# Nablax/Path-Tracer-CUDA-OpenGL

Measured on AMD Instinct MI355X. Metric: Mray/s + ms/frame, bunny-in-Cornell 1920×1080 @1024spp, 1/2/4/8 MI355X, higher is better.
Workload: dtype f32

## Files before the change

### path-tracer-cuda-opengl_amd/csrc/pt_device.hip

```cpp
#include <hip/hip_runtime.h>

#include <algorithm>
#include <array>
#include <atomic>
#include <chrono>
#include <cfloat>
#include <cmath>
#include <cstdio>
#include <cstdlib>
#include <cstring>
#include <limits>
#include <type_traits>
#include <memory>
#include <string>
#include <vector>

#include "../host/pt_denoise_dev.hpp"
#include "../host/pt_error.hpp"
#include "../host/pt_host.hpp"
#include "../host/pt_inst_dev.hpp"
#include "../host/pt_instancing.hpp"
#include "../host/pt_wide8.hpp"
#include "../host/pt_wide_dev.hpp"
#include "pt.h"
// ... 74 lines not shown
    if (l == 0.0f) return f3(0.0f, 0.0f, 0.0f);
    return divs(v, l);
}
__device__ __forceinline__ float3 xyz(float4 v) { return f3(v.x, v.y, v.z); }

struct Xorwow {
    uint32_t d, v0, v1, v2, v3, v4;
    __device__ __forceinline__ uint32_t next() {
        uint32_t t = v0 ^ (v0 >> 2);
        v0 = v1; v1 = v2; v2 = v3; v3 = v4;
        v4 = __builtin_amdgcn_bitop3_b32(v4, v4 << 4, t ^ (t << 1), 0x96);
        d += 362437u;
        return v4 + d;
    }
    __device__ __forceinline__ float uniform() { return uniformOf(next()); }
    __device__ __forceinline__ float centered2() { return centered2Of(uniform()); }
    __device__ __forceinline__ float3 centered2x3() {
        uint32_t t0 = v0 ^ (v0 >> 2), t1 = v1 ^ (v1 >> 2), t2 = v2 ^ (v2 >> 2);
        asm volatile("" : "+v"(t0), "+v"(t1), "+v"(t2));
        uint32_t r0, r1;
        asm volatile("v_mov_b32 %0, %1" : "=v"(r0) : "v"(v3));
        asm volatile("v_mov_b32 %0, %1" : "=v"(r1) : "v"(v4));
        const uint32_t n0 = __builtin_amdgcn_bitop3_b32(v4, v4 << 4, t0 ^ (t0 << 1), 0x96);
        const uint32_t n1 = __builtin_amdgcn_bitop3_b32(n0, n0 << 4, t1 ^ (t1 << 1), 0x96);
        const uint32_t n2 = __builtin_amdgcn_bitop3_b32(n1, n1 << 4, t2 ^ (t2 << 1), 0x96);
        uint32_t x0 = n0 + (d + 362437u), x1 = n1 + (d + 2u * 362437u);
        asm volatile("" : "+v"(x0), "+v"(x1));
        d += 3u * 362437u;
        v0 = r0; v1 = r1; v2 = n0; v3 = n1; v4 = n2;
        return f3(centered2Of(uniformOf(x0)), centered2Of(uniformOf(x1)), centered2Of(uniformOf(n2 + d)));
    }
};

__device__ __forceinline__ Xorwow sampleStream(uint32_t k0, uint32_t k1, uint32_t sample, uint32_t pixel) {
    uint32_t c0 = sample, c1 = pixel, c2 = 0u, c3 = 0x53414D50u;
#pragma unroll 2
    for (int r = 0; r < 10; r++) {
        const uint64_t p0 = (uint64_t)0xD2511F53u * c0, p1 = (uint64_t)0xCD9E8D57u * c2;
        const uint32_t hi0 = (uint32_t)(p0 >> 32), lo0 = (uint32_t)p0;
        const uint32_t hi1 = (uint32_t)(p1 >> 32), lo1 = (uint32_t)p1;
        const uint32_t n0 = __builtin_amdgcn_bitop3_b32(hi1, c1, k0, 0x96), n2 = __builtin_amdgcn_bitop3_b32(hi0, c3, k1, 0x96);
        c0 = n0; c1 = lo1; c2 = n2; c3 = lo0;
        k0 += 0x9E3779B9u;
        k1 += 0xBB67AE85u;
    }
    return Xorwow{c3, c0, c1, c2, c3 ^ 0x6C078965u, c0 ^ c1 ^ 0x2545F491u};
}

struct SlabHit { bool hit; float lo; };

__host__ __device__ constexpr int nodeBoxIdx(int child, int axis, int isMax) { return 6 * child + 2 * axis + isMax; }

typedef float v2f __attribute__((ext_vector_type(2)));

__device__ __forceinline__ SlabHit slabPair(v2f X, v2f Y, v2f Z, float3 o, float3 inv, float tmin, float tmax) {
    const v2f tx = (X - o.x) * inv.x, ty = (Y - o.y) * inv.y, tz = (Z - o.z) * inv.z;
    float nx = inv.x < 0.0f ? tx.y : tx.x, fx = inv.x < 0.0f ? tx.x : tx.y;
    float ny = inv.y < 0.0f ? ty.y : ty.x, fy = inv.y < 0.0f ? ty.x : ty.y;
    float nz = inv.z < 0.0f ? tz.y : tz.x, fz = inv.z < 0.0f ? tz.x : tz.y;
    float lo = fmaxf(fmaxf(fmaxf(tmin, nx), ny), nz);
    float hi = fminf(fminf(fminf(tmax, fx), fy), fz);
    return SlabHit{!(hi < lo), lo};
}
struct SlabHit2 { SlabHit l, r; };
__device__ __forceinline__ SlabHit2 slabBoth(float4 a, float4 b, float4 q, float3 o, float3 inv, float tmin,
                                             float tmax) {
    const v2f lx = (v2f{a.x, a.y} - o.x) * inv.x, ly = (v2f{a.z, a.w} - o.y) * inv.y,
              lz = (v2f{b.x, b.y} - o.z) * inv.z;
    const v2f rx = (v2f{b.z, b.w} - o.x) * inv.x, ry = (v2f{q.x, q.y} - o.y) * inv.y,
              rz = (v2f{q.z, q.w} - o.z) * inv.z;
// ... 3 lines not shown
        const float lo = fmaxf(fmaxf(fmaxf(tmin, sx ? lx.y : lx.x), sy ? ly.y : ly.x), sz ? lz.y : lz.x);
        const float hi = fminf(fminf(fminf(tmax, sx ? lx.x : lx.y), sy ? ly.x : ly.y), sz ? lz.x : lz.y);
        h.l = SlabHit{!(hi < lo), lo};
    }
    {
        const float lo = fmaxf(fmaxf(fmaxf(tmin, sx ? rx.y : rx.x), sy ? ry.y : ry.x), sz ? rz.y : rz.x);
        const float hi = fminf(fminf(fminf(tmax, sx ? rx.x : rx.y), sy ? ry.x : ry.y), sz ? rz.x : rz.y);
        h.r = SlabHit{!(hi < lo), lo};
    }
    return h;
}
__device__ __forceinline__ SlabHit slabLeft(float4 a, float4 b, float3 o, float3 inv, float tmin, float tmax) {
    return slabPair(v2f{a.x, a.y}, v2f{a.z, a.w}, v2f{b.x, b.y}, o, inv, tmin, tmax);
}
__device__ __forceinline__ SlabHit slabRight(float4 b, float4 q, float3 o, float3 inv, float tmin, float tmax) {
    return slabPair(v2f{b.z, b.w}, v2f{q.x, q.y}, v2f{q.z, q.w}, o, inv, tmin, tmax);
}

struct Prim { float4 p0, p1, p2; };
__device__ __forceinline__ __amdgpu_buffer_rsrc_t rawRsrc(const void* base) {
    return __builtin_amdgcn_make_buffer_rsrc(const_cast<void*>(base), 0, -1 , 0x00020000);
}
template <int S>
__device__ __forceinline__ uint32_t shlOpaque(uint32_t x) {
    uint32_t t;
    asm("v_lshlrev_b32 %0, %1, %2" : "=v"(t) : "i"(S), "v"(x));
    return t;
}
__device__ __forceinline__ uint32_t mul80(uint32_t x) {
    if constexpr (pt::kW8NodeDwords == 32) return x << 7;
    return shlOpaque<6>(x) + (x << 4);
}
__device__ __forceinline__ uint32_t mul48(uint32_t x) { return shlOpaque<5>(x) + (x << 4); }
__device__ __forceinline__ float4 bload4(__amdgpu_buffer_rsrc_t r, uint32_t off) {
    return __builtin_bit_cast(float4, __builtin_amdgcn_raw_buffer_load_b128(r, off, 0, 0));
}

__device__ __forceinline__ Prim loadPrim(const DevScene& S, uint32_t k) {
    const float4* p = S.prims + 3 * (size_t)k;
    return Prim{p[0], p[1], p[2]};
}

__device__ __forceinline__ float primHitT(const Prim& q, bool sphere, float3 o, float3 d, float tmin, float closest) {
    if (sphere) {
        float3 oc = sub(o, xyz(q.p0));
        float r = q.p1.x;
        float a = len2(d);
        float half_b = dot3(oc, d);
        float cc = len2(oc) - r * r;
        float disc = half_b * half_b - a * cc;
        if (disc < 0.0f) return -1.0f;
        float sq = sqrtf(disc);
        float root = (-half_b - sq) / a;
        if (root < tmin || closest < root) {
            root = (-half_b + sq) / a;
            if (root < tmin || closest < root) return -1.0f;
        }
        return root;
    }
    const float3 v0 = xyz(q.p0);
    float3 e1 = sub(xyz(q.p1), v0), e2 = sub(xyz(q.p2), v0);
    float3 s1 = cross3(d, e2);
    float det = dot3(s1, e1);
    if (det == 0.0f) return -1.0f;
    float3 s = sub(o, v0);
    float3 s2 = cross3(s, e1);
// ... 74 lines not shown
                                         int& best, float& bestLo, bool leafBoxes, bool& redo, uint32_t keyHi = 0u) {
    const bool sph = SPH && __float_as_uint(q.p2.w) != 0u;
    const float t = primHitAny(q, sph, o, d, tmin);
    if (t >= 0.0f) {
        const int k = (int)(keyHi | __float_as_uint(q.p0.w));
        const bool none = best < 0, bSph = SPH && (best & (int)kSphereBit) != 0;
        const int bk = SPH ? best & (int)kPrimMask : best;
        const bool tie = sph ? (none || !bSph || k > bk) : (!none && !bSph && k < bk);
        redo = redo || (t >= closest && t < bestLo);
        if (t < closest || (t == closest && tie)) {
            bool take = true;
            float lo = -__builtin_inff();
            if (leafBoxes) {
                const SlabHit b = refLeafBox(q, sph, o, inv, tmin, __builtin_inff());
                take = b.hit && !(closest < b.lo);
                redo = redo || (b.hit && closest < b.lo);
                lo = t < b.lo ? b.lo : lo;
            }
            if (take) {
                closest = t;
                best = k | (sph ? (int)kSphereBit : 0);
                bestLo = lo;
            }
        }
    }
}

__device__ __forceinline__ float rcpRNWave(float x, uint64_t hasM) {
    if constexpr (!PT_FAST_RCP) return 1.0f / x;
    const uint32_t ex = (__float_as_uint(x) >> 23) & 0xffu;
    const uint64_t slowM = hasM & __ballot(ex - kRcpExpLo > kRcpExpHi - kRcpExpLo);
    float y = rcpNewton(x);
    if (__builtin_expect(slowM != 0, 0)) y = __builtin_amdgcn_inverse_ballot_w64(slowM) ? 1.0f / x : y;
    return y;
}
__device__ __forceinline__ void wideTestTri(const Prim& q, uint64_t hasM, float3 o, float3 d, float tmin, float& closest,
                                            int& best, float& t2) {
    const float3 v0 = xyz(q.p0), e1 = xyz(q.p1), e2 = xyz(q.p2);
    const float3 s1 = cross3(d, e2);
    const float det = dot3(s1, e1);
    const float3 s = sub(o, v0);
    const float3 s2 = cross3(s, e1);
    const float inv = rcpRNWave(det, hasM);
    const float t = dot3(s2, e2) * inv;
    const float b1 = dot3(s1, s) * inv;
    const float b2 = dot3(s2, d) * inv;
    const int k = (int)__float_as_uint(q.p0.w);
    const uint64_t rejM = __ballot(b1 >= 1.0f) | __ballot(b1 <= 0.0f) | __ballot(b2 >= 1.0f) | __ballot(b2 <= 0.0f) |
                          __ballot(b1 + b2 >= 1.0f);
    const uint64_t hitM = hasM & __ballot(det != 0.0f) & __ballot(t > tmin) & ~rejM;
    const uint64_t takeM = hitM & (__ballot(t < closest) | (__ballot(t == closest) & __ballot(k < best)));
    const float mid = __builtin_amdgcn_fmed3f(t, closest, t2);
    t2 = __builtin_amdgcn_inverse_ballot_w64(hitM) ? mid : t2;
    closest = __builtin_amdgcn_inverse_ballot_w64(takeM) ? t : closest;
    best = __builtin_amdgcn_inverse_ballot_w64(takeM) ? k : best;
}
__device__ __forceinline__ bool deferredRedo(float4 xy, float2 z, float3 o, float3 inv, float closest, float t2) {
    const SlabHit b = slabPair(v2f{xy.x, xy.y}, v2f{xy.z, xy.w}, v2f{z.x, z.y}, o, inv, 0.001f, __builtin_inff());
    return !b.hit || (closest < b.lo && t2 < b.lo);
}

template <bool MIX = false, bool DEC3 = false>
__device__ __forceinline__ uint32_t wideHits(uint4 n0, uint4 n1, uint4 n2, uint4 n3, uint4 n4, float3 o, float3 inv,
                                             uint32_t oct, float tmin, float tmax) {
    constexpr uint32_t kMixExp = MIX ? 24u : 0u;
    float ax, ay, az;
// ... 179 lines not shown
        const uint32_t lref = __float_as_uint(r.x), rref = __float_as_uint(r.y);
        int next = -1;
        if (from < 0) {
            const SlabHit hl = slabLeft(a, b, o, inv, tmin, closest);
            if (hl.hit && (lref & kLeafBit)) {
                const float t = primHitT(loadPrim(S, lref & kPrimMask), (lref & kSphereBit) != 0, o, d, tmin, closest);
                if (t >= 0.0f) { closest = t; best = (int)(lref & kPrimMask); }
            }
            const SlabHit hr = slabRight(b, q, o, inv, tmin, closest);
            if (hr.hit && (rref & kLeafBit)) {
                const float t = primHitT(loadPrim(S, rref & kPrimMask), (rref & kSphereBit) != 0, o, d, tmin, closest);
                if (t >= 0.0f) { closest = t; best = (int)(rref & kPrimMask); }
            }
            if (hr.hit && !(rref & kLeafBit)) next = (int)rref;
            else if (!(lref & kLeafBit) && slabLeft(a, b, o, inv, tmin, closest).hit) next = (int)lref;
        } else if ((uint32_t)from == rref && !(lref & kLeafBit) && slabLeft(a, b, o, inv, tmin, closest).hit) {
            next = (int)lref;
        }
        if (next >= 0) {
            node = next;
            from = -1;
        } else {
            if (node == 0) { finished = true; break; }
            from = node;
            node = S.iparent[node];
        }
    }
    if (!finished) atomicOr(S.err, 4u);
    return best;
}

struct HitRec { float3 p, n; int mat, obj; bool front; float4 m0; float ir; int type; };

__device__ __forceinline__ HitRec makeHitFrom(const float4* shade, int k, float t, float3 o, float3 d) {
    HitRec h;
    const float4* r = shade + 3 * (size_t)k;
    const float4 s0 = r[0], s1 = r[1], s2 = r[2];
    const uint32_t tf = __float_as_uint(s2.y);
    h.p = add(o, scale(t, d));
    float3 outward;
    if (tf >> 16) {
        outward = divs(sub(h.p, xyz(s0)), s0.w);
    } else {
        outward = xyz(s0);
    }
    h.front = dot3(d, outward) < 0.0f;
    h.n = h.front ? outward : neg(outward);
    h.mat = (int)__float_as_uint(s2.z);
    h.obj = (int)__float_as_uint(s2.w);
    h.m0 = s1;
    h.ir = s2.x;
    h.type = (int)(tf & 0xffffu);
    return h;
}
__device__ __forceinline__ HitRec makeHit(const DevScene& S, int k, float t, float3 o, float3 d) {
    return makeHitFrom(S.shade, k, t, o, d);
}

__device__ __forceinline__ float3 xformPoint(float4 r0, float4 r1, float4 r2, float3 p) {
    return f3(((r0.x * p.x + r0.y * p.y) + r0.z * p.z) + r0.w, ((r1.x * p.x + r1.y * p.y) + r1.z * p.z) + r1.w,
              ((r2.x * p.x + r2.y * p.y) + r2.z * p.z) + r2.w);
}
__device__ __forceinline__ float3 xformDir(float4 r0, float4 r1, float4 r2, float3 v) {
    return f3((r0.x * v.x + r0.y * v.y) + r0.z * v.z, (r1.x * v.x + r1.y * v.y) + r1.z * v.z,
              (r2.x * v.x + r2.y * v.y) + r2.z * v.z);
}
__device__ __forceinline__ HitRec makeHitInst(const DevScene& S, uint32_t key, float t, float3 o, float3 d, int& obj) {
    const uint32_t inst = key >> S.gBits, g = key & ((1u << S.gBits) - 1u);
    const float4* ir = S.winst + 4 * (size_t)inst;
    const float4 r0 = ir[0], r1 = ir[1], r2 = ir[2], ex = ir[3];
    const float4* r = S.wshade + 3 * (size_t)g;
    const float4 s0 = r[0], s1 = r[1], s2 = r[2];
    const uint32_t tf = __float_as_uint(s2.y);
    const bool ident = __float_as_uint(ex.y) == 1u, linIdent = __float_as_uint(ex.y) != 0u;
    HitRec h;
    h.p = add(o, scale(t, d));
    float3 outward;
// ... 569 lines not shown
        } else if (bidT < ks) { slice = bidT % P.splitWays; bidT /= P.splitWays; }
        else bidT -= ks - P.splitTiles;
    }
    int tile = (SAMPLE || crit) ? -1 : tileOf(P, bidT), nSamples = SAMPLE ? 0 : P.spp;
    int col = 0, lrow = 0;
    bool valid = false;
    uint32_t idx = 0u;
    if constexpr (!SAMPLE) {
        if (crit) {
            const int k = bidT * P.critLanes + lane;
            valid = lane < P.critLanes && k < P.nCrit;
            idx = valid ? P.critList[k] : 0u;
            col = (int)(idx % (uint32_t)P.width);
            lrow = (int)(idx / (uint32_t)P.width);
        } else {
            col = (tile % P.tiles_x) * 8 + (lane & 7);
            lrow = (tile / P.tiles_x) * 8 + (lane >> 3);
            valid = col < P.width && lrow < P.nrows && (slice < 0 || (lane * P.splitWays) / kWave == slice);
            idx = valid ? (uint32_t)lrow * (uint32_t)P.width + (uint32_t)col : 0u;
            if (CRITK && valid && P.critFlag && P.critFlag[idx]) valid = false;
        }
    }
    const unsigned long long tStart = __builtin_amdgcn_s_memrealtime();
    if (!SAMPLE && !crit && bidT < P.prioTiles) {
        if (P.prioLevel >= 3) __builtin_amdgcn_s_setprio(3);
        else if (P.prioLevel == 2) __builtin_amdgcn_s_setprio(2);
        else __builtin_amdgcn_s_setprio(1);
    }
    float fcol = (float)col;
    float frow = valid ? (float)globalRow(lrow, P.stripe_h, P.nparts, P.part) : 0.0f;
    const DevScene& S = P.S;
    const __amdgpu_buffer_rsrc_t nodeRsrc = rawRsrc(WIDE ? (const void*)S.wnodes : (const void*)S.nodes);
    uint32_t* my = stk + lane;
    uint32_t sRays = 0, sVisits = 0, sTris = 0, sSph = 0, sPaths = 0;
#ifdef PT_DIAG
    uint32_t itN = 0, itL = 0, itS = 0, sPops = 0, sRedo = 0;
    uint32_t sRedoMiss = 0;
    unsigned long long sSpecN = 0, sIdleN = 0;
    unsigned long long sHalf = 0, sParkT = 0;
    unsigned long long cycN = 0, cycL = 0, cycS = 0, cycH = 0;
    unsigned long long cycSh = 0, cycTk = 0, cycNp = 0, cycBr = 0;
#define PT_DIAG_ADD(v, x) (v) += (x)
#else
#define PT_DIAG_ADD(v, x) ((void)0)
#endif

    Xorwow g{};
    if constexpr (!SAMPLE) {
        if (valid) g = Xorwow{P.sd[idx], P.s0[idx], P.s1[idx], P.s2[idx], P.s3[idx], P.s4[idx]};
    }
    float3 sum = f3(0.0f, 0.0f, 0.0f), o = f3(0.0f, 0.0f, 0.0f), d = f3(0.0f, 0.0f, 1.0f);
    float3 inv = d, att = f3(1.0f, 1.0f, 1.0f);
    float closest = 0.0f;
    int best = -1, depthLeft = 0, sample = 0, node = -1, sp = 0, qn = 0;
    constexpr int LQ = (SAMPLE && !WIDE && STACK <= 32) ? PT_LEAF_QUEUE_SAMPLE : kLeafQ;
    uint32_t qref[LQ];
    float lq[LQ];
#pragma unroll
    for (int i = 0; i < LQ; i++) { qref[i] = 0u; lq[i] = 0.0f; }
    uint32_t ng = 0u, tgBase = 0u, tg = 0u, oct = 0u;
    float bestLo = 0.0f;
    const uint64_t allM = __ballot(true);
    uint64_t activeM = 0;
    uint32_t depthPaths = 0;
    uint32_t pxRays = 0;
    uint64_t needTaskM = SAMPLE ? allM : 0;
    uint32_t poolBase = 0u, poolLeft = 0u;


#define PT_BEGIN_RAY(SH)                                                                            \
    do {                                                                                          \
        const bool sh_ = NEE && (SH);                                                             \
        if constexpr (NEE) depthLeft -= sh_ ? 0 : 1;                                              \
        else depthLeft--;                                                                         \
        if constexpr (SAMPLE) {    \
            if (kargs()->measureCost)                                                             \
                __hip_atomic_fetch_add(&taskState[lane].w, 1u, __ATOMIC_RELAXED, __HIP_MEMORY_SCOPE_WORKGROUP); \
        }                                                                                         \
        closest = sh_ ? kShadowTmax : __builtin_inff();                                           \
        best = -1;                                                                                \
        sp = 0;                                                                                   \
        qn = 0;                                                                                   \
        if constexpr (CRITK) pxRays++;                                                            \
        if constexpr (WIDE) {                 \
            inv = f3(rcpRN(d.x), rcpRN(d.y), rcpRN(d.z));                                         \
            const uint32_t oc_ = (inv.x < 0.0f ? 1u : 0u) | (inv.y < 0.0f ? 2u : 0u) | (inv.z < 0.0f ? 4u : 0u); \
            oct = oc_;                                                                            \
            tg = 0u;                                                                              \
                    \
                   \
            if constexpr (TRI) bestLo = closest;                                                  \
            else bestLo = INST || kargs()->S.hasSpheres ? -__builtin_inff() : closest;            \
            ng = S.nprims > 0 ? (1u << oc_) : 0u;                                                 \
                 \
            if (!INST && ((kargs()->camFar && !sh_ && depthLeft + 1 == kargs()->max_depth) ||      \
                          (PT_WIDE_MIX && mixUnsafe(inv, kargs()->S.mixLim)))) {                   \
                ng = 0u;             \
                oct |= 8u;      \
            }                                                                                     \
            if (INST && kargs()->camFar && !sh_ && depthLeft + 1 == kargs()->max_depth) {          \
                     \
                const auto& K_ = *kargs();                                                        \
                (void)instEntry(K_.S.cx, K_.S.cy, K_.S.cz, K_.S.ext, o, d, inv);                   \
            }                                                                                     \
            if (CRITK && crit) PT_CRIT_TRACE();                                                    \
        } else if (S.nprims <= 1) {                                                               \
            node = -1;                                                                            \
            if (S.nprims == 1) {        \
                const float t1 = primHitT(loadPrim(S, 0), __float_as_uint(S.prims[2].w) != 0, o, d, \
                                          0.001f, closest);                                       \
                if (t1 >= 0.0f) { closest = t1; best = 0; }                                       \
            }                                                                                     \
        } else {                                                                                  \
            inv = f3(rcpRN(d.x), rcpRN(d.y), rcpRN(d.z));                                         \
            node = 0;                                                                             \
        }                                                                                         \
    } while (0)
#define PT_CRIT_TRACE()                                                                             \
    do {                                                                                          \
        const bool lb_ = S.nprims > 1;                                                            \
        bool sph_ = false;                                                                        \
        if constexpr (!TRI) sph_ = kargs()->S.hasSpheres != 0;                                    \
        bool redo_ = false;                                                                       \
        for (;;) {                                                                                \
            while (tg) {                                                                          \
                const uint32_t k_ = tgBase + (uint32_t)__builtin_ctz(tg);                         \
                tg &= tg - 1u;                                                                    \
                const float4* w_ = reinterpret_cast<const float4*>(reinterpret_cast<const char*>(S.wprims) + mul48(k_)); \
                const Prim q_{w_[0], w_[1], w_[2]};                                               \
                if constexpr (TRI) {                                 \
                    sTris += (uint32_t)__popcll(__ballot(true));                                  \
                    wideTestTri(q_, __ballot(true), o, d, 0.001f, closest, best, bestLo);         \
                } else {                                                                          \
                const bool isS_ = __float_as_uint(q_.p2.w) != 0u;                                 \
                sTris += (uint32_t)__popcll(__ballot(!isS_));                                     \
                sSph += (uint32_t)__popcll(__ballot(isS_));                                       \
                if (sph_) wideTest<true>(q_, o, d, inv, 0.001f, closest, best, bestLo, lb_, redo_, 0u); \
                else if (INST) wideTest<false>(q_, o, d, inv, 0.001f, closest, best, bestLo, lb_, redo_, 0u); \
                else wideTestTri(q_, __ballot(true), o, d, 0.001f, closest, best, bestLo);    \
                }                                                                                 \
            }                                                                                     \
            if ((ng & 0xffu) == 0u) {                                                             \
                if (sp == 0) break;                                                               \
                sp--;                                                                             \
                ng = my[sp * kWave];                                                              \
            }                                                                                     \
            const uint32_t bit_ = (uint32_t)__builtin_ctz(ng & 0xffu);                            \
            const uint32_t child_ = (ng >> 8) + (bit_ ^ (oct & 7u));                              \
            ng &= ~(1u << bit_);                                                                  \
            if (ng & 0xffu) { my[sp * kWave] = ng; sp++; }    \
            sVisits += (uint32_t)__popcll(__ballot(true));                                        \
            const uint32_t off_ = mul80(child_);                                                  \
            const uint4 n0_ = __builtin_bit_cast(uint4, __builtin_amdgcn_raw_buffer_load_b128(nodeRsrc, off_, 0, 0)); \
            const uint4 n1_ = __builtin_bit_cast(uint4, __builtin_amdgcn_raw_buffer_load_b128(nodeRsrc, off_ + 16u, 0, 0)); \
            const uint4 n2_ = __builtin_bit_cast(uint4, __builtin_amdgcn_raw_buffer_load_b128(nodeRsrc, off_ + 32u, 0, 0)); \
            const uint4 n3_ = __builtin_bit_cast(uint4, __builtin_amdgcn_raw_buffer_load_b128(nodeRsrc, off_ + 48u, 0, 0)); \
            const uint4 n4_ = __builtin_bit_cast(uint4, __builtin_amdgcn_raw_buffer_load_b128(nodeRsrc, off_ + 64u, 0, 0)); \
            const uint32_t h_ = wideHits<PT_WIDE_MIX != 0>(n0_, n1_, n2_, n3_, n4_, o, inv, oct & 7u, 0.001f, closest); \
            ng = (n1_.x << 8) | (h_ >> 24);                                                      \
            tgBase = n1_.y;                                                                       \
            tg = h_ & 0xffffffu;                                                                  \
        }                                                                                         \
        if (redo_) oct |= 8u;              \
    } while (0)
#define PT_TAKE_TASKS(got)                                                                          \
    do {                                                                                          \
        const auto& Q_ = *kargs();                                                                \
        for (;;) {                                                                                \
            const uint64_t m_ = needTaskM;                                                        \
            if (m_ == 0) break;                                                                   \
            if (poolLeft == 0u) {  \
                const int leader_ = __ffsll((unsigned long long)m_) - 1;                          \
                          \
                const uint32_t grab_ = (uint32_t)kTaskPool;                                       \
                uint32_t b_ = 0;                                                                  \
                if (lane == leader_) b_ = atomicAdd(Q_.taskCounter, grab_);                       \
                poolBase = __builtin_amdgcn_readfirstlane((uint32_t)__shfl((int)b_, leader_));    \
                poolLeft = grab_;                                                                 \
            }                                                                                     \
              \
            const uint32_t base_ = poolBase;                                                      \
            const uint32_t take_ = min((uint32_t)__popcll(m_), poolLeft);                         \
            poolBase += take_;                                                                    \
            poolLeft -= take_;                                                                    \
            const uint32_t g0_ = base_ >> 6, off_ = base_ & 63u;                                  \
            const uint32_t slotA_ = Q_.nblocksShift >= 0 ? g0_ >> Q_.nblocksShift : g0_ / (uint32_t)Q_.ngroups; \
            const uint32_t blkA_ = g0_ - slotA_ * (uint32_t)Q_.ngroups;                           \
            const bool wrap_ = blkA_ + 1u == (uint32_t)Q_.ngroups;                                  \
            const uint32_t slotB_ = wrap_ ? slotA_ + 1u : slotA_, blkB_ = wrap_ ? 0u : blkA_ + 1u; \
            const uint32_t nslots_ = (uint32_t)Q_.ntiles;                                          \
             \
                                                    \
            const uint32_t xyA_ = slotA_ < nslots_ ? ((KU32)Q_.tileXY)[__builtin_amdgcn_readfirstlane(slotA_)] : 0u; \
            const uint32_t xyB_ = slotB_ < nslots_ ? ((KU32)Q_.tileXY)[__builtin_amdgcn_readfirstlane(slotB_)] : 0u; \
            const uint32_t txA_ = xyA_ & 0xffffu, tyA_ = xyA_ >> 16;                              \
            const uint32_t txB_ = xyB_ & 0xffffu, tyB_ = xyB_ >> 16;                              \
            const uint32_t k_ = (uint32_t)__popcll(m_ & ((1ull << lane) - 1ull));                 \
            const uint32_t o_ = off_ + k_, px_ = o_ & 63u;                                        \
            const bool hi_ = o_ >= 64u;                                                           \
            const int c_ = (int)((hi_ ? txB_ : txA_) * 8u + (px_ & 7u));                          \
            const int r_ = (int)((hi_ ? tyB_ : tyA_) * 8u + (px_ >> 3));                          \
            const uint64_t took_ = m_ & __ballot(k_ < take_);                                     \
            const uint64_t left_ = took_ & __ballot(base_ + k_ < Q_.ntasks);                      \
            const uint64_t in_ = left_ & __ballot(c_ < Q_.width) & __ballot(r_ < Q_.nrows);       \
            needTaskM &= ~((took_ & ~left_) | in_);                                               \
            got |= in_;                                                                           \
            if (laneOf(in_)) {                                                                    \
                const uint32_t s0_ = (hi_ ? blkB_ : blkA_) * (uint32_t)Q_.span;                   \
                taskState[lane] = make_uint4((uint32_t)c_ | ((uint32_t)r_ << 16), s0_,             \
                                             min(s0_ + (uint32_t)Q_.span, (uint32_t)Q_.spp), 0u); \
                sum = f3(0.0f, 0.0f, 0.0f);                                                       \
            }                                                                                     \
        }                                                                                         \
    } while (0)
#define PT_FINISH_TASK(ts)                                                                          \
    do {                                                                                          \
        unsigned long long* acc_ = kargs()->pixAcc + 4 * (size_t)(((ts).x >> 16) * (uint32_t)kargs()->width + ((ts).x & 0xffffu)); \
        addBlock(acc_, sum, (ts).w + 1u, kargs()->measureCost != 0);                              \
    } while (0)
#define PT_NEW_PATH()                                                                               \
    do {                                                                                          \
        const auto& Q_ = *kargs();                                                                \
        if constexpr (SAMPLE) {                   \
            const uint4 ts_ = taskState[lane];                                                    \
            fcol = (float)(ts_.x & 0xffffu);                                                      \
            const uint32_t grow_ = (uint32_t)globalRowFast((int)(ts_.x >> 16), Q_.stripe_h, Q_.stripeShift, \
                                                           Q_.nparts, Q_.part);                  \
            frow = (float)grow_;                                                                  \
            g = sampleStream(Q_.seed0, Q_.seed1, Q_.sampleBase + ts_.y,                           \
                             grow_ * (uint32_t)Q_.width + (ts_.x & 0xffffu));                      \
        }                                                                                         \
        const float u_ = (fcol + g.uniform()) * Q_.invW;                                           \
        const float v_ = (frow + g.uniform()) * Q_.invH;                                           \
        o = ld3(Q_.cam.pos);                                                                            \
        d = sub(add(add(ld3(Q_.cam.ll), scale(u_, ld3(Q_.cam.hor))), scale(v_, ld3(Q_.cam.ver))), ld3(Q_.cam.pos));       \
        if (Q_.cam.lens != 0.0f) lensOffset(ld3(Q_.cam.right), ld3(Q_.cam.up), Q_.cam.lens, g, o, d); \
        att = f3(1.0f, 1.0f, 1.0f);                                                               \
        depthLeft = Q_.max_depth;                                                                  \
        if constexpr (NEE) {                                     \
            neeV[0 * kWave + lane] = 0.0f; neeV[1 * kWave + lane] = 0.0f; neeV[2 * kWave + lane] = 0.0f; \
            neeF[lane] = 0u;                                                                      \
        }                                                                                         \
    } while (0)

#define PT_SKY() skyK<LIT>(d, att)

    bool started = false;
    if constexpr (SAMPLE) {
        if (P.max_depth <= 0) {
            for (;;) {
                uint64_t got = 0;
                PT_TAKE_TASKS(got);
                if (got == 0) break;
                needTaskM |= got;
                if (laneOf(got)) {
                    uint4 ts = taskState[lane];
                    depthPaths += ts.z - ts.y;
                    while (ts.y < ts.z) {
                        taskState[lane].y = ts.y;
                        PT_NEW_PATH();
                        sum = add(sum, endOf<NEE>(f3(0.0f, 0.0f, 0.0f), PT_SKY()));
                        ts.y++;
                        if (ts.y < ts.z) (void)kargs();
                    }
                    PT_FINISH_TASK(ts);
                }
            }
            needTaskM = 0;
            waveReduceAdd(P.counters + 4, depthPaths);
        }
    } else if (valid) {
        if (P.max_depth <= 0) {
            for (; sample < nSamples; sample++) {
                PT_NEW_PATH();
                sum = add(sum, endOf<NEE>(f3(0.0f, 0.0f, 0.0f), PT_SKY()));
            }
        } else if (nSamples > 0) {
            PT_NEW_PATH();
            PT_BEGIN_RAY(false);
            started = true;
        }
    }
    activeM = __ballot(started);
    sRays += (uint32_t)__popcll(activeM);
    sPaths += (uint32_t)__popcll(activeM) +
              (!SAMPLE && P.max_depth <= 0 ? (uint32_t)__popcll(__ballot(valid)) * (uint32_t)nSamples : 0u);

    for (;;) {
#ifdef PT_DIAG
        const unsigned long long tH0 = __builtin_amdgcn_s_memtime();
#endif
        uint64_t mN, mL, mS;
        if constexpr (WIDE) {
            const uint64_t noPrims = __ballot(tg == 0u);
            const uint64_t nodesLeft = __ballot(((ng & 0xffu) | (uint32_t)sp) != 0u);
            uint64_t mayVisit = noPrims;
            if constexpr (SPEC)
                mayVisit |= __ballot(SPECN == 1 ? (oct & 48u) == 0u : ((oct >> 4) & 3u) < (uint32_t)SPECN);
            mN = mayVisit & nodesLeft;
            mL = allM & ~noPrims;
            mS = (activeM & noPrims & ~nodesLeft) | needTaskM;
        } else {
            const uint64_t inTree = __ballot(node >= 0), queued = __ballot(qn > 0);
            mN = inTree & (LQ == 2 ? allM & ~queued : __ballot(qn <= LQ - 2));
            mL = queued;
            mS = (activeM & ~inTree & ~queued) | needTaskM;
        }
        if ((mN | mL | mS) == 0) break;
        const int nN = __popcll(mN), nL = __popcll(mL), nS = __popcll(mS);
        int kind;
        if (nN == 0) kind = nL > 0 ? 1 : 2;
        else if (nL >= P.leafBatch) kind = 1;
        else if (nS >= P.shadeBatch) kind = 2;
        else if (!SAMPLE && nN < P.nodeMin && (nL | nS)) kind = nL >= nS ? 1 : 2;
        else kind = 0;
#ifdef PT_DIAG
        const unsigned long long tK0 = __builtin_amdgcn_s_memtime();
        cycH += tK0 - tH0;
#endif

        if (kind == 0) {
            sVisits += (uint32_t)nN;
            PT_DIAG_ADD(itN, 1u);
            const bool wantNode = laneOf(mN);
            if constexpr (WIDE) {
                PT_DIAG_ADD(sSpecN, (unsigned long long)__popcll(__ballot(tg != 0u && ((ng & 0xffu) != 0u || sp > 0))));
                PT_DIAG_ADD(sIdleN, (unsigned long long)(64 - nN));
            }
            if constexpr (INST) {
                if (wantNode) {
                    while ((ng & 0xffu) == 0u && sp > 0) {
                        sp--;
                        ng = my[sp * kWave];
                        if (ng == kInstMarker) {
                            o = f3(wray[0 * kWave + lane], wray[1 * kWave + lane], wray[2 * kWave + lane]);
                            if (oct & 8u) {
                                d = f3(wray[3 * kWave + lane], wray[4 * kWave + lane], wray[5 * kWave + lane]);
                                inv = f3(rcpRN(d.x), rcpRN(d.y), rcpRN(d.z));
                                oct = (inv.x < 0.0f ? 1u : 0u) | (inv.y < 0.0f ? 2u : 0u) | (inv.z < 0.0f ? 4u : 0u);
                            } else {
                                oct &= 7u;
                            }
                            ng = 0u;
                        }
                    }
                    if (ng & 0xffu) {
                        const uint32_t bit = (uint32_t)__builtin_ctz(ng & 0xffu);
                        const uint32_t child = (ng >> 8) + (bit ^ (oct & 7u));
                        ng &= ~(1u << bit);
                        if (ng & 0xffu) { my[sp * kWave] = ng; sp++; }
                        uint32_t off = mul80(child);
                        uint4 n0 = __builtin_bit_cast(uint4, __builtin_amdgcn_raw_buffer_load_b128(nodeRsrc, off, 0, 0));
                        uint4 n1 = __builtin_bit_cast(uint4, __builtin_amdgcn_raw_buffer_load_b128(nodeRsrc, off + 16u, 0, 0));
                        uint4 n2 = __builtin_bit_cast(uint4, __builtin_amdgcn_raw_buffer_load_b128(nodeRsrc, off + 32u, 0, 0));
                        uint4 n3 = __builtin_bit_cast(uint4, __builtin_amdgcn_raw_buffer_load_b128(nodeRsrc, off + 48u, 0, 0));
// ... 120 lines not shown
                    node = -1;
                }
            }
        }
        if (kind == 1) {
            bool tested = false, sph = false;
            PT_DIAG_ADD(itL, 1u);
            if constexpr (WIDE) {
                PT_DIAG_ADD(sPops, (uint32_t)nL);
                uint32_t k0 = 0u, k1 = 0u;
                const bool h0 = laneOf(mL);
                if (h0) k0 = tgBase + (uint32_t)__builtin_ctz(tg);
                tg &= tg - 1u;
                const uint64_t m1 = __ballot((int)tg > 0);
                const bool h1 = laneOf(m1);
                if (h1) k1 = tgBase + (uint32_t)__builtin_ctz(tg);
                tg &= tg - 1u;
                const float4* w0 = reinterpret_cast<const float4*>(reinterpret_cast<const char*>(S.wprims) + mul48(k0));
                const float4* w1 = reinterpret_cast<const float4*>(reinterpret_cast<const char*>(S.wprims) + mul48(k1));
                const Prim q0{w0[0], w0[1], w0[2]}, q1{w1[0], w1[1], w1[2]};
                bool redo = false;
#ifdef PT_DIAG
                {
                    sHalf += (unsigned long long)__popcll(__ballot(h0 && !h1));
                    const bool pk = !INST && (oct & 64u) != 0u;
                    sParkT += (unsigned long long)(__popcll(__ballot(pk && h0)) + __popcll(__ballot(pk && h1)));
                }
#endif
                const bool lb = !INST && S.nprims > 1;
                const uint32_t kh = INST ? (oct >> 8) << kargs()->S.gBits : 0u;
                if constexpr (TRI) {
                    wideTestTri(q0, mL, o, d, 0.001f, closest, best, bestLo);
                    wideTestTri(q1, m1, o, d, 0.001f, closest, best, bestLo);
                    sTris += (uint32_t)nL + (uint32_t)__popcll(m1);
                } else if (kargs()->S.hasSpheres) {
                    if (h0) wideTest<true>(q0, o, d, inv, 0.001f, closest, best, bestLo, lb, redo, kh);
                    if (h1) wideTest<true>(q1, o, d, inv, 0.001f, closest, best, bestLo, lb, redo, kh);
                    const uint64_t s0 = mL & __ballot(__float_as_uint(q0.p2.w) != 0u);
                    const uint64_t s1 = m1 & __ballot(__float_as_uint(q1.p2.w) != 0u);
                    sTris += (uint32_t)nL + (uint32_t)__popcll(m1) - (uint32_t)__popcll(s0) - (uint32_t)__popcll(s1);
                    sSph += (uint32_t)__popcll(s0) + (uint32_t)__popcll(s1);
                } else {
                    if constexpr (INST) {
                        if (h0) wideTest<false>(q0, o, d, inv, 0.001f, closest, best, bestLo, lb, redo, kh);
                        if (h1) wideTest<false>(q1, o, d, inv, 0.001f, closest, best, bestLo, lb, redo, kh);
                    } else {
                        wideTestTri(q0, mL, o, d, 0.001f, closest, best, bestLo);
                        wideTestTri(q1, m1, o, d, 0.001f, closest, best, bestLo);
                    }
                    sTris += (uint32_t)nL + (uint32_t)__popcll(m1);
                }
                if (redo) oct |= 8u;
                if (SPEC && tg == 0u && (oct & 48u)) {
                    oct -= 16u;
                    const uint32_t c = SPECN == 1 ? 0u : (oct >> 4) & 3u;
                    tgBase = pend[(2u * c) * kWave + lane];
                    tg = pend[(2u * c + 1u) * kWave + lane];
#ifdef PT_DIAG
                    oct |= 64u;
#endif
                }
            } else {
            PT_DIAG_ADD(sPops, (uint32_t)nL);
            Prim pf0{}, pf1{};
            if (qn > 0) pf0 = loadPrim(S, qref[0] & kPrimMask);
            if (qn > 1) pf1 = loadPrim(S, qref[1] & kPrimMask);
#pragma unroll
            for (int k_ = 0; k_ < LQ; k_++) {
                const bool act = qn > 0;
                if (__ballot(act) == 0) break;
                tested = false;
                sph = false;
            if (act) {
                const uint32_t ref = qref[0];
                const float lo = lq[0];
#pragma unroll
                for (int i = 0; i + 1 < LQ; i++) { qref[i] = qref[i + 1]; lq[i] = lq[i + 1]; }
                qn--;
                const uint32_t k = ref & kPrimMask;
                sph = (ref & kSphereBit) != 0;
                if (!(closest < lo)) {
                    const Prim pr = k_ == 0 ? pf0 : (k_ == 1 ? pf1 : loadPrim(S, k));
                    {
                        tested = true;
                        const float t = primHitT(pr, sph, o, d, 0.001f, closest);
                        if (t >= 0.0f) { closest = t; best = (int)k; }
                    }
                }
            }
            sTris += (uint32_t)__popcll(__ballot(tested && !sph));
            sSph += (uint32_t)__popcll(__ballot(tested && sph));
            }
            }
        }
        if (kind == 2) {
            const uint64_t shadeM = mS & ~needTaskM;
            const bool shading = laneOf(shadeM);
            uint32_t nf = 0u;
            if constexpr (NEE) nf = neeF[lane];
            const bool shadowQ = NEE && (nf & 1u) != 0u;
            if constexpr (WIDE && !INST) {
                bool redo = shading && (oct & 8u);
#ifdef PT_DIAG
                bool missed = false;
#endif
                bool triScene = TRI;
                if constexpr (!TRI) triScene = !kargs()->S.hasSpheres;
                if (triScene && S.nprims > 1) {
                    if (shading && best >= 0 && !redo) {
                        const float4* bx = kargs()->S.wbox + 2 * (size_t)best;
                        redo = deferredRedo(bx[0], *reinterpret_cast<const float2*>(bx + 1), o, inv, closest, bestLo);
#ifdef PT_DIAG
                        {
                            const float2 bz_ = *reinterpret_cast<const float2*>(bx + 1);
                            const float4 bx_ = bx[0];
                            missed = !slabPair(v2f{bx_.x, bx_.y}, v2f{bx_.z, bx_.w}, v2f{bz_.x, bz_.y}, o, inv, 0.001f,
                                               __builtin_inff()).hit;
                        }
#endif
                    }
                }
                PT_DIAG_ADD(sRedo, (uint32_t)__popcll(__ballot(redo)));
                PT_DIAG_ADD(sRedoMiss, (uint32_t)__popcll(__ballot(missed)));
                if (redo) {
                    const DevScene S2 = ldScene(kargs());
                    closest = shadowQ ? kShadowTmax : __builtin_inff();
                    const int k = traceRefStackless(S2, o, d, 0.001f, closest);
                    best = k >= 0 ? (int)S2.rankOf[k] : -1;
                }
            }
            PT_DIAG_ADD(itS, 1u);
            bool done = false;
            bool shadowNow = false;
            if (shading) {
                float3 contrib = f3(0.0f, 0.0f, 0.0f);
                bool wasShadow = false;
                if constexpr (NEE) {
                    if (shadowQ) {
                        if (best < 0) {
                            neeV[0 * kWave + lane] += neeV[3 * kWave + lane];
                            neeV[1 * kWave + lane] += neeV[4 * kWave + lane];
                            neeV[2 * kWave + lane] += neeV[5 * kWave + lane];
                        }
                        d = f3(neeV[6 * kWave + lane], neeV[7 * kWave + lane], neeV[8 * kWave + lane]);
                        neeF[lane] = nf & ~1u;
                        wasShadow = true;
                    }
                }
                if (wasShadow) {
                } else if (best < 0) {
                    contrib = PT_SKY();
                    done = true;
                } else {
                    int objI_;
                    HitRec h = INST ? makeHitInst(ldScene(kargs()), (uint32_t)best & kPrimMask, closest, o, d, objI_)
                                    : (WIDE ? makeHitFrom(kargs()->S.wshade, best & (int)kPrimMask, closest, o, d)
                                            : makeHit(S, best, closest, o, d));
                    if (!scatterInto(h, d, att, g)) {
                        if constexpr (LIT) contrib = emitted(h, att);
                        if constexpr (NEE) {
                            const int sk = INST ? best & ((1 << kargs()->S.gBits) - 1) : best & (int)kPrimMask;
                            if ((nf & 2u) && sampledLight(kargs()->S.wshade, sk, h)) {
                                if constexpr (MIS && INST)
                                    contrib = emittedWeightedAt(kargs()->lights,
                                                                instLightSlot(kargs()->instLightFirst, kargs()->lightSlot,
                                                                              (uint32_t)best & kPrimMask, kargs()->S.gBits),
                                                                kargs()->nLights, closest, d, neeV[9 * kWave + lane], contrib);
                                else if constexpr (MIS)
                                    contrib = emittedWeighted(kargs()->lights, kargs()->lightSlot, kargs()->nLights, h.obj,
                                                              closest, d, neeV[9 * kWave + lane], contrib);
                                else contrib = f3(0.0f, 0.0f, 0.0f);
                            }
                        }
                        done = true;
                    } else {
                        o = h.p;
                        if (depthLeft == 0) { contrib = PT_SKY(); done = true; }
                        else if constexpr (NEE) {
                            nf &= ~2u;
                            if (h.type == PT_LAMBERTIAN) {
                                nf |= 2u;
                                float3 w, term;
                                if constexpr (MIS) neeV[9 * kWave + lane] = scatterPdf(h.n, d);
                                if (lightSample<MIS>(kargs()->lights, kargs()->nLights, o, h.n, att, g, w, term)) {
                                    neeV[3 * kWave + lane] = term.x; neeV[4 * kWave + lane] = term.y; neeV[5 * kWave + lane] = term.z;
                                    neeV[6 * kWave + lane] = d.x; neeV[7 * kWave + lane] = d.y; neeV[8 * kWave + lane] = d.z;
                                    d = w;
                                    nf |= 1u;
                                    shadowNow = true;
// ... 18 lines not shown
                finM = doneM & __ballot(y1 == ts.z);
                if (laneOf(finM)) PT_FINISH_TASK(ts);
                needTaskM |= finM;
            } else {
                const int s1 = sample + (done ? 1 : 0);
                doneM = shadeM & __ballot(s1 != sample);
                finM = doneM & __ballot(s1 == nSamples);
                sample = s1;
            }
            activeM &= ~finM;
            uint64_t newRayM = shadeM & ~finM, newSampleM = doneM & ~finM;
#ifdef PT_DIAG
            const unsigned long long tS1 = __builtin_amdgcn_s_memtime();
#endif
            if constexpr (SAMPLE) {
                uint64_t got = 0;
                PT_TAKE_TASKS(got);
                activeM |= got;
                newRayM |= got;
                newSampleM |= got;
            }
#ifdef PT_DIAG
            const unsigned long long tS2 = __builtin_amdgcn_s_memtime();
#endif
            if (laneOf(newSampleM)) PT_NEW_PATH();
#ifdef PT_DIAG
            const unsigned long long tS3 = __builtin_amdgcn_s_memtime();
#endif
            if (laneOf(newRayM)) PT_BEGIN_RAY(shadowNow);
#ifdef PT_DIAG
            const unsigned long long tS4 = __builtin_amdgcn_s_memtime();
            cycSh += tS1 - tK0; cycTk += tS2 - tS1; cycNp += tS3 - tS2; cycBr += tS4 - tS3;
#endif
            sRays += (uint32_t)__popcll(newRayM);
            sPaths += (uint32_t)__popcll(newSampleM);
        }
#ifdef PT_DIAG
        {
            const unsigned long long dK = __builtin_amdgcn_s_memtime() - tK0;
            if (kind == 0) cycN += dK;
            else if (kind == 1) cycL += dK;
            else cycS += dK;
        }
#endif
    }
    if constexpr (!SAMPLE) {
        if (valid) {
            storePixel(P, idx, sum);
            P.sd[idx] = g.d; P.s0[idx] = g.v0; P.s1[idx] = g.v1; P.s2[idx] = g.v2; P.s3[idx] = g.v3; P.s4[idx] = g.v4;
            if (CRITK && P.pixRays) P.pixRays[idx] = pxRays;
        }
    }
    const unsigned long long tEnd = __builtin_amdgcn_s_memrealtime();
    if (!SAMPLE && !crit && lane == 0) atomicMax(P.tileCost + tile, (unsigned)min(tEnd - tStart, 0xffffffffull));
    if (P.waveTimes && lane == 0) {
        unsigned xcc;
        asm volatile("s_getreg_b32 %0, hwreg(HW_REG_XCC_ID)" : "=s"(xcc));
        P.waveTimes[3 * (size_t)blockIdx.x + 0] = tStart;
        P.waveTimes[3 * (size_t)blockIdx.x + 1] = tEnd;
        P.waveTimes[3 * (size_t)blockIdx.x + 2] = (unsigned long long)tile | ((unsigned long long)(xcc & 0xf) << 32);
    }
    if (lane == 0) {
        atomicAdd(P.counters + 0, (unsigned long long)sRays);
        atomicAdd(P.counters + 1, (unsigned long long)sVisits);
        atomicAdd(P.counters + 2, (unsigned long long)sTris);
        atomicAdd(P.counters + 3, (unsigned long long)sSph);
        atomicAdd(P.counters + 4, (unsigned long long)sPaths);
#ifdef PT_DIAG
        atomicAdd(P.counters + 8, (unsigned long long)itN);
        atomicAdd(P.counters + 9, (unsigned long long)itL);
        atomicAdd(P.counters + 10, (unsigned long long)itS);
        atomicAdd(P.counters + 11, (unsigned long long)sPops);
        atomicAdd(P.counters + 12, cycN);
        atomicAdd(P.counters + 13, cycL);
        atomicAdd(P.counters + 14, cycS);
        atomicAdd(P.counters + 15, cycH);
        atomicAdd(P.counters + 16, cycSh);
        atomicAdd(P.counters + 17, cycTk);
        atomicAdd(P.counters + 18, cycNp);
        atomicAdd(P.counters + 19, cycBr);
        atomicAdd(P.counters + 20, (unsigned long long)sRedo);
        atomicAdd(P.counters + 21, sSpecN);
        atomicAdd(P.counters + 22, sIdleN);
        atomicAdd(P.counters + 23, (unsigned long long)sRedoMiss);
        atomicAdd(P.counters + 25, sHalf);
        atomicAdd(P.counters + 27, sParkT);
#endif
    }
}
#undef PT_BEGIN_RAY
#undef PT_CRIT_TRACE
#undef PT_NEW_PATH
#undef PT_SKY
#undef PT_TAKE_TASKS
#undef PT_FINISH_TASK
#undef PT_DIAG_ADD

#ifdef PT_TU_COMPAT
}

namespace pt {
template <int S, bool TRI>
static void launchCompatWideTri(const RenderParams& P, hipStream_t st) {
    const int grid = P.compatGrid;
    if (P.nLights > 0 && P.mis) renderKernelWF<S, false, true, false, true, true, true, TRI><<<grid, kWave, 0, st>>>(P);
    else if (P.nLights > 0) renderKernelWF<S, false, true, false, true, true, false, TRI><<<grid, kWave, 0, st>>>(P);
    else if (P.lit) renderKernelWF<S, false, true, false, true, false, false, TRI><<<grid, kWave, 0, st>>>(P);
    else renderKernelWF<S, false, true, false, false, false, false, TRI><<<grid, kWave, 0, st>>>(P);
}
int launchCompatWide(int stack, const void* params, hipStream_t st) {
    const RenderParams& P = *static_cast<const RenderParams*>(params);
    switch (stack) {
#define PT_COMPAT_WIDE(S)                                                                    \
        case S:                                                                                  \
            P.tri ? launchCompatWideTri<S, true>(P, st) : launchCompatWideTri<S, false>(P, st);   \
            break;
        PT_COMPAT_WIDE(8)
        PT_COMPAT_WIDE(16)
        PT_COMPAT_WIDE(24)
#undef PT_COMPAT_WIDE
        default: return -1;
    }
    return 0;
}
template <bool TRI>
static const void* compatWideKernel(int stack) {
    return stack == 8 ? reinterpret_cast<const void*>(&renderKernelWF<8, false, true, false, false, false, false, TRI>)
         : stack == 16 ? reinterpret_cast<const void*>(&renderKernelWF<16, false, true, false, false, false, false, TRI>)
         : stack == 24 ? reinterpret_cast<const void*>(&renderKernelWF<24, false, true, false, false, false, false, TRI>) : nullptr;
// ... 2779 lines not shown
```

Measured before the change: 23240.

## Peel RNG rounds, wave-ballot reciprocal, scalar counters, and trim hit-record work

```diff
diff --git a/path-tracer-cuda-opengl_amd/csrc/pt_device.hip b/path-tracer-cuda-opengl_amd/csrc/pt_device.hip
--- a/path-tracer-cuda-opengl_amd/csrc/pt_device.hip
+++ b/path-tracer-cuda-opengl_amd/csrc/pt_device.hip
@@ -130,10 +130,24 @@
     }
 };
 
+template <bool PEEL = false>
 __device__ __forceinline__ Xorwow sampleStream(uint32_t k0, uint32_t k1, uint32_t sample, uint32_t pixel) {
     uint32_t c0 = sample, c1 = pixel, c2 = 0u, c3 = 0x53414D50u;
-#pragma unroll 2
-    for (int r = 0; r < 10; r++) {
+    if constexpr (PEEL) {
+        const uint64_t p0 = (uint64_t)0xD2511F53u * sample;
+        const uint32_t a0 = pixel ^ k0, a2 = __builtin_amdgcn_bitop3_b32((uint32_t)(p0 >> 32), 0x53414D50u, k1, 0x96);
+        k0 += 0x9E3779B9u;
+        k1 += 0xBB67AE85u;
+        const uint64_t q0 = (uint64_t)0xD2511F53u * a0, q1 = (uint64_t)0xCD9E8D57u * a2;
+        c0 = (uint32_t)(q1 >> 32) ^ k0;
+        c1 = (uint32_t)q1;
+        c2 = __builtin_amdgcn_bitop3_b32((uint32_t)(q0 >> 32), (uint32_t)p0, k1, 0x96);
+        c3 = (uint32_t)q0;
+        k0 += 0x9E3779B9u;
+        k1 += 0xBB67AE85u;
+    }
+#pragma unroll(PEEL ? 8 : 2)
+    for (int r = PEEL ? 2 : 0; r < 10; r++) {
         const uint64_t p0 = (uint64_t)0xD2511F53u * c0, p1 = (uint64_t)0xCD9E8D57u * c2;
         const uint32_t hi0 = (uint32_t)(p0 >> 32), lo0 = (uint32_t)p0;
         const uint32_t hi1 = (uint32_t)(p1 >> 32), lo1 = (uint32_t)p1;
@@ -203,6 +217,9 @@
     return shlOpaque<6>(x) + (x << 4);
 }
 __device__ __forceinline__ uint32_t mul48(uint32_t x) { return shlOpaque<5>(x) + (x << 4); }
+__device__ __forceinline__ void waveCount(uint32_t& acc, uint32_t n) {
+    asm("s_add_u32 %0, %0, %1" : "+s"(acc) : "s"(n) : "scc");
+}
 __device__ __forceinline__ float4 bload4(__amdgpu_buffer_rsrc_t r, uint32_t off) {
     return __builtin_bit_cast(float4, __builtin_amdgcn_raw_buffer_load_b128(r, off, 0, 0));
 }
@@ -343,6 +360,20 @@
     const uint64_t slowM = hasM & __ballot(ex - kRcpExpLo > kRcpExpHi - kRcpExpLo);
     float y = rcpNewton(x);
     if (__builtin_expect(slowM != 0, 0)) y = __builtin_amdgcn_inverse_ballot_w64(slowM) ? 1.0f / x : y;
+    return y;
+}
+constexpr uint32_t kRcpKeyLim = (255u - kRcpExpHi + kRcpExpLo) << 24;
+__device__ __forceinline__ uint32_t rcpKey(float x) { return (__float_as_uint(x) << 1) + ((255u - kRcpExpHi) << 24); }
+__device__ __forceinline__ float3 rcpRN3Wave(float3 d) {
+    if constexpr (!PT_FAST_RCP) return f3(1.0f / d.x, 1.0f / d.y, 1.0f / d.z);
+    const uint32_t kx = rcpKey(d.x), ky = rcpKey(d.y), kz = rcpKey(d.z);
+    const uint64_t slowM = __ballot(min(min(kx, ky), kz) < kRcpKeyLim);
+    float3 y = f3(rcpNewton(d.x), rcpNewton(d.y), rcpNewton(d.z));
+    if (__builtin_expect(slowM != 0, 0)) {
+        y.x = kx < kRcpKeyLim ? 1.0f / d.x : y.x;
+        y.y = ky < kRcpKeyLim ? 1.0f / d.y : y.y;
+        y.z = kz < kRcpKeyLim ? 1.0f / d.z : y.z;
+    }
     return y;
 }
 __device__ __forceinline__ void wideTestTri(const Prim& q, uint64_t hasM, float3 o, float3 d, float tmin, float& closest,
@@ -588,17 +619,16 @@
 
 struct HitRec { float3 p, n; int mat, obj; bool front; float4 m0; float ir; int type; };
 
+template <bool SPH = true>
 __device__ __forceinline__ HitRec makeHitFrom(const float4* shade, int k, float t, float3 o, float3 d) {
     HitRec h;
-    const float4* r = shade + 3 * (size_t)k;
+    const float4* r = reinterpret_cast<const float4*>(reinterpret_cast<const char*>(shade) + mul48((uint32_t)k));
     const float4 s0 = r[0], s1 = r[1], s2 = r[2];
     const uint32_t tf = __float_as_uint(s2.y);
     h.p = add(o, scale(t, d));
-    float3 outward;
-    if (tf >> 16) {
-        outward = divs(sub(h.p, xyz(s0)), s0.w);
-    } else {
-        outward = xyz(s0);
+    float3 outward = xyz(s0);
+    if constexpr (SPH) {
+        if (tf >> 16) outward = divs(sub(h.p, xyz(s0)), s0.w);
     }
     h.front = dot3(d, outward) < 0.0f;
     h.n = h.front ? outward : neg(outward);
@@ -1234,6 +1264,12 @@
     const DevScene& S = P.S;
     const __amdgpu_buffer_rsrc_t nodeRsrc = rawRsrc(WIDE ? (const void*)S.wnodes : (const void*)S.nodes);
     uint32_t* my = stk + lane;
+    constexpr bool CTU = !SAMPLE && WIDE && !INST;
+#define PT_COUNT(v, x)                                                                              \
+    do {                                                                                          \
+        if constexpr (CTU) (v) += (x);                                                            \
+        else waveCount((v), (x));                                                                 \
+    } while (0)
     uint32_t sRays = 0, sVisits = 0, sTris = 0, sSph = 0, sPaths = 0;
 #ifdef PT_DIAG
     uint32_t itN = 0, itL = 0, itS = 0, sPops = 0, sRedo = 0;
@@ -1285,7 +1321,8 @@
         qn = 0;                                                                                   \
         if constexpr (CRITK) pxRays++;                                                            \
         if constexpr (WIDE) {                 \
-            inv = f3(rcpRN(d.x), rcpRN(d.y), rcpRN(d.z));                                         \
+            if constexpr (CTU) inv = f3(rcpRN(d.x), rcpRN(d.y), rcpRN(d.z));                      \
+            else inv = rcpRN3Wave(d);                                                             \
             const uint32_t oc_ = (inv.x < 0.0f ? 1u : 0u) | (inv.y < 0.0f ? 2u : 0u) | (inv.z < 0.0f ? 4u : 0u); \
             oct = oc_;                                                                            \
             tg = 0u;                                                                              \
@@ -1331,12 +1368,12 @@
                 const float4* w_ = reinterpret_cast<const float4*>(reinterpret_cast<const char*>(S.wprims) + mul48(k_)); \
                 const Prim q_{w_[0], w_[1], w_[2]};                                               \
                 if constexpr (TRI) {                                 \
-                    sTris += (uint32_t)__popcll(__ballot(true));                                  \
+                    PT_COUNT(sTris, (uint32_t)__popcll(__ballot(true)));                          \
                     wideTestTri(q_, __ballot(true), o, d, 0.001f, closest, best, bestLo);         \
                 } else {                                                                          \
                 const bool isS_ = __float_as_uint(q_.p2.w) != 0u;                                 \
-                sTris += (uint32_t)__popcll(__ballot(!isS_));                                     \
-                sSph += (uint32_t)__popcll(__ballot(isS_));                                       \
+                PT_COUNT(sTris, (uint32_t)__popcll(__ballot(!isS_)));                             \
+                PT_COUNT(sSph, (uint32_t)__popcll(__ballot(isS_)));                               \
                 if (sph_) wideTest<true>(q_, o, d, inv, 0.001f, closest, best, bestLo, lb_, redo_, 0u); \
                 else if (INST) wideTest<false>(q_, o, d, inv, 0.001f, closest, best, bestLo, lb_, redo_, 0u); \
                 else wideTestTri(q_, __ballot(true), o, d, 0.001f, closest, best, bestLo);    \
@@ -1351,7 +1388,7 @@
             const uint32_t child_ = (ng >> 8) + (bit_ ^ (oct & 7u));                              \
             ng &= ~(1u << bit_);                                                                  \
             if (ng & 0xffu) { my[sp * kWave] = ng; sp++; }    \
-            sVisits += (uint32_t)__popcll(__ballot(true));                                        \
+            PT_COUNT(sVisits, (uint32_t)__popcll(__ballot(true)));                                \
             const uint32_t off_ = mul80(child_);                                                  \
             const uint4 n0_ = __builtin_bit_cast(uint4, __builtin_amdgcn_raw_buffer_load_b128(nodeRsrc, off_, 0, 0)); \
             const uint4 n1_ = __builtin_bit_cast(uint4, __builtin_amdgcn_raw_buffer_load_b128(nodeRsrc, off_ + 16u, 0, 0)); \
@@ -1408,7 +1445,9 @@
             needTaskM &= ~((took_ & ~left_) | in_);                                               \
             got |= in_;                                                                           \
             if (laneOf(in_)) {                                                                    \
-                const uint32_t s0_ = (hi_ ? blkB_ : blkA_) * (uint32_t)Q_.span;                   \
+                  \
+                const uint32_t sA_ = blkA_ * (uint32_t)Q_.span, sB_ = blkB_ * (uint32_t)Q_.span;  \
+                const uint32_t s0_ = hi_ ? sB_ : sA_;                                             \
                 taskState[lane] = make_uint4((uint32_t)c_ | ((uint32_t)r_ << 16), s0_,             \
                                              min(s0_ + (uint32_t)Q_.span, (uint32_t)Q_.spp), 0u); \
                 sum = f3(0.0f, 0.0f, 0.0f);                                                       \
@@ -1417,7 +1456,8 @@
     } while (0)
 #define PT_FINISH_TASK(ts)                                                                          \
     do {                                                                                          \
-        unsigned long long* acc_ = kargs()->pixAcc + 4 * (size_t)(((ts).x >> 16) * (uint32_t)kargs()->width + ((ts).x & 0xffffu)); \
+         \
+        unsigned long long* acc_ = kargs()->pixAcc + 4 * (size_t)(__umul24((ts).x >> 16, (uint32_t)kargs()->width) + ((ts).x & 0xffffu)); \
         addBlock(acc_, sum, (ts).w + 1u, kargs()->measureCost != 0);                              \
     } while (0)
 #define PT_NEW_PATH()                                                                               \
@@ -1429,7 +1469,7 @@
             const uint32_t grow_ = (uint32_t)globalRowFast((int)(ts_.x >> 16), Q_.stripe_h, Q_.stripeShift, \
                                                            Q_.nparts, Q_.part);                  \
             frow = (float)grow_;                                                                  \
-            g = sampleStream(Q_.seed0, Q_.seed1, Q_.sampleBase + ts_.y,                           \
+            g = sampleStream<true>(Q_.seed0, Q_.seed1, Q_.sampleBase + ts_.y,                     \
                              grow_ * (uint32_t)Q_.width + (ts_.x & 0xffffu));                      \
         }                                                                                         \
         const float u_ = (fcol + g.uniform()) * Q_.invW;                                           \
@@ -1484,9 +1524,9 @@
         }
     }
     activeM = __ballot(started);
-    sRays += (uint32_t)__popcll(activeM);
-    sPaths += (uint32_t)__popcll(activeM) +
-              (!SAMPLE && P.max_depth <= 0 ? (uint32_t)__popcll(__ballot(valid)) * (uint32_t)nSamples : 0u);
+    PT_COUNT(sRays, (uint32_t)__popcll(activeM));
+    PT_COUNT(sPaths, (uint32_t)__popcll(activeM) +
+                                 (!SAMPLE && P.max_depth <= 0 ? (uint32_t)__popcll(__ballot(valid)) * (uint32_t)nSamples : 0u));
 
     for (;;) {
 #ifdef PT_DIAG
@@ -1522,7 +1562,7 @@
 #endif
 
         if (kind == 0) {
-            sVisits += (uint32_t)nN;
+            PT_COUNT(sVisits, (uint32_t)nN);
             PT_DIAG_ADD(itN, 1u);
             const bool wantNode = laneOf(mN);
             if constexpr (WIDE) {
@@ -1709,14 +1749,14 @@
                 if constexpr (TRI) {
                     wideTestTri(q0, mL, o, d, 0.001f, closest, best, bestLo);
                     wideTestTri(q1, m1, o, d, 0.001f, closest, best, bestLo);
-                    sTris += (uint32_t)nL + (uint32_t)__popcll(m1);
+                    PT_COUNT(sTris, (uint32_t)nL + (uint32_t)__popcll(m1));
                 } else if (kargs()->S.hasSpheres) {
                     if (h0) wideTest<true>(q0, o, d, inv, 0.001f, closest, best, bestLo, lb, redo, kh);
                     if (h1) wideTest<true>(q1, o, d, inv, 0.001f, closest, best, bestLo, lb, redo, kh);
                     const uint64_t s0 = mL & __ballot(__float_as_uint(q0.p2.w) != 0u);
                     const uint64_t s1 = m1 & __ballot(__float_as_uint(q1.p2.w) != 0u);
-                    sTris += (uint32_t)nL + (uint32_t)__popcll(m1) - (uint32_t)__popcll(s0) - (uint32_t)__popcll(s1);
-                    sSph += (uint32_t)__popcll(s0) + (uint32_t)__popcll(s1);
+                    PT_COUNT(sTris, (uint32_t)nL + (uint32_t)__popcll(m1) - (uint32_t)__popcll(s0) - (uint32_t)__popcll(s1));
+                    PT_COUNT(sSph, (uint32_t)__popcll(s0) + (uint32_t)__popcll(s1));
                 } else {
                     if constexpr (INST) {
                         if (h0) wideTest<false>(q0, o, d, inv, 0.001f, closest, best, bestLo, lb, redo, kh);
@@ -1725,7 +1765,7 @@
                         wideTestTri(q0, mL, o, d, 0.001f, closest, best, bestLo);
                         wideTestTri(q1, m1, o, d, 0.001f, closest, best, bestLo);
                     }
-                    sTris += (uint32_t)nL + (uint32_t)__popcll(m1);
+                    PT_COUNT(sTris, (uint32_t)nL + (uint32_t)__popcll(m1));
                 }
                 if (redo) oct |= 8u;
                 if (SPEC && tg == 0u && (oct & 48u)) {
@@ -1765,8 +1805,8 @@
                     }
                 }
             }
-            sTris += (uint32_t)__popcll(__ballot(tested && !sph));
-            sSph += (uint32_t)__popcll(__ballot(tested && sph));
+            PT_COUNT(sTris, (uint32_t)__popcll(__ballot(tested && !sph)));
+            PT_COUNT(sSph, (uint32_t)__popcll(__ballot(tested && sph)));
             }
             }
         }
@@ -1785,7 +1825,8 @@
                 if constexpr (!TRI) triScene = !kargs()->S.hasSpheres;
                 if (triScene && S.nprims > 1) {
                     if (shading && best >= 0 && !redo) {
-                        const float4* bx = kargs()->S.wbox + 2 * (size_t)best;
+                        const float4* bx = reinterpret_cast<const float4*>(reinterpret_cast<const char*>(kargs()->S.wbox) +
+                                                                           ((uint32_t)best << 5));
                         redo = deferredRedo(bx[0], *reinterpret_cast<const float2*>(bx + 1), o, inv, closest, bestLo);
 #ifdef PT_DIAG
                         {
@@ -1831,7 +1872,7 @@
                 } else {
                     int objI_;
                     HitRec h = INST ? makeHitInst(ldScene(kargs()), (uint32_t)best & kPrimMask, closest, o, d, objI_)
-                                    : (WIDE ? makeHitFrom(kargs()->S.wshade, best & (int)kPrimMask, closest, o, d)
+                                    : (WIDE ? makeHitFrom<!TRI>(kargs()->S.wshade, best & (int)kPrimMask, closest, o, d)
                                             : makeHit(S, best, closest, o, d));
                     if (!scatterInto(h, d, att, g)) {
                         if constexpr (LIT) contrib = emitted(h, att);
@@ -1916,8 +1957,8 @@
             const unsigned long long tS4 = __builtin_amdgcn_s_memtime();
             cycSh += tS1 - tK0; cycTk += tS2 - tS1; cycNp += tS3 - tS2; cycBr += tS4 - tS3;
 #endif
-            sRays += (uint32_t)__popcll(newRayM);
-            sPaths += (uint32_t)__popcll(newSampleM);
+            PT_COUNT(sRays, (uint32_t)__popcll(newRayM));
+            PT_COUNT(sPaths, (uint32_t)__popcll(newSampleM));
         }
 #ifdef PT_DIAG
         {
@@ -1979,6 +2020,7 @@
 #undef PT_TAKE_TASKS
 #undef PT_FINISH_TASK
 #undef PT_DIAG_ADD
+#undef PT_COUNT
 
 #ifdef PT_TU_COMPAT
 }
```

After: 23650 (median of 6 runs). 1.8% higher.
